# apple/ml-mdm

Hardware: AMD Instinct MI355X
Metric: denoise-steps/sec, whole job = N x optimizer steps/s at per-GPU batch 64 (train fwd+bwd+optimizer, cc12m_64x64 U-Net) (higher is better)
Workload: dtype bf16; 1 GPU; unet64 train step, per-GPU batch 64, global batch 64; global_batch=64, parallelism=dp1, settle_steps=15

## Files before the change

### include/mdm_hip_ext.h

```cpp
#ifndef MDM_HIP_EXT_H_
#define MDM_HIP_EXT_H_
#ifdef __cplusplus
extern "C" {
#endif

int mdm_attn_cross_bias(const void* qkv, const void* kvc, const float* mask, const float* bias, int bias_ld,
                        const void* base, int base_ld, void* out, int B, int L, int S, int H, int d, int dtype,
                        void* stream);

int mdm_attn_cross_maps(const void* qkv, const void* kvc, const float* mask, const float* bias, int bias_ld, float* acc,
                        int acc_ld, float w_host, const float* w_dev, int B, int L, int S, int H, int d, int dtype,
                        void* stream);

int mdm_attn_cross_maps_bwd(const void* qkv, const void* kvc, const float* mask, const float* dacc, int dacc_ld, float w,
                            void* dq, size_t dq_bs, int dq_rs, int B, int L, int S, int H, int d, int dtype, void* stream);

int mdm_freeu_plan(int N, int H, int W, int C1, int C2, int dtype, int structure, size_t* ws_bytes);
int mdm_freeu_stats(const void* h, const void* r, void* ws, size_t ws_bytes, int N, int H, int W, int C1, int C2,
                    int structure, int dtype, void* stream);
int mdm_freeu_apply(const void* h, const void* r, const void* ws, size_t ws_bytes, void* out, int N, int H, int W, int C1,
                    int C2, float b, float s, int structure, int dtype, void* stream);

int mdm_cfg_plan(int B, size_t chw, int rescale_on, size_t* ws_bytes);
int mdm_cfg_stats(const float* x_t, const float* pred, const float* pred_uncond, const float* gamma, const float* run_prev,
// ... 10 lines not shown

int mdm_abs_quantile_plan(int B, size_t n, size_t* ws_bytes);
int mdm_abs_quantile(const float* x, void* ws, size_t ws_bytes, int B, size_t n, float q, float cmin, float cmax, float* thr,
                     float* stats, void* stream);

int mdm_t5_attn_fwd_lse(const void* qkv, const int* seq_start, const int* pos, const float* bias_table, void* out, float* lse,
                        int B, int T, int S, int max_len, int H, int d, int dtype, void* stream);
int mdm_t5_attn_bwd(const void* qkv, const void* out, const float* lse, const void* dout, const int* seq_start, const int* pos,
                    const float* bias_table, void* dqkv, int B, int T, int S, int max_len, int H, int d, int dtype,
                    void* stream);
int mdm_t5_gated_gelu_bwd(const void* u, const void* dy, void* du, int T, int F, int dtype, void* stream);
int mdm_t5_rms_bwd(const float* x, const float* ln_w, const void* dh, float* dx, void* dx_lo, int T, int D, float eps,
                   int dtype, void* stream);
int mdm_t5_final_rms_bwd(const float* x, const void* delta, const float* ln_w, const float* dout, const int* flat, float* dx,
                         void* dx_lo, int T, int D, float eps, int dtype, void* stream);
int mdm_t5_embed_rms_slots(const int* ids, const float* table, const int* slot_of_id, const float* learned, const float* ln_w,
                           float* x, void* h, int T, int D, int vocab, int n_ids, int P, float eps, int dtype, void* stream);
int mdm_t5_embed_bwd(const float* dx0, const int* slot_start, const int* tokens, float* dlearned, int P, int D, int n, int T,
                     void* stream);

int mdm_sampler_step_sa(const float* x_t, const float* pred, const float* pred_uncond, float guidance, const float* gamma,
                        const float* gamma_last, const float* gamma_h0, const float* gamma_h1, const float* gate,
                        const float* thr, const float* noise, const unsigned long long* rng_state, int rng_stream, float* h0,
                        float* h1, float* psum, float* x0_out, float* x_last_out, int B, size_t chw, int pred_type, int clip,
                        float image_scale, int max_predictor, int max_corrector, void* stream);

int mdm_sampler_invert_step(const float* x_s, const float* pred, const float* pred_uncond, float guidance,
                            const float* gamma_s, const float* gamma_t, float* x_t_out, int B, size_t chw, int pred_type,
                            void* stream);
int mdm_sampler_noise_map(const float* x_t, const float* x_s, const float* pred, const float* pred_uncond, float guidance,
                          const float* gamma, const float* gamma_last, const float* thr, float* z_out, int B, size_t chw,
                          int pred_type, int mode, float ddim_eta, int clip, float image_scale, void* stream);

#ifdef __cplusplus
}
#endif
#endif
```

### ml-mdm_amd/csrc/gemm_conv.hip

```cpp
#include <stdio.h>
#include <stdlib.h>

#include <type_traits>
#include <utility>

#include "common.hpp"
#include "conv_args.hpp"

namespace mdm {



__device__ __forceinline__ void load4(const float* p, float (&o)[4]) {
  const f32x4 t = *reinterpret_cast<const f32x4*>(p);
  o[0] = t[0]; o[1] = t[1]; o[2] = t[2]; o[3] = t[3];
}
__device__ __forceinline__ void load4(const bf16* p, float (&o)[4]) {
  const bf16x4 t = *reinterpret_cast<const bf16x4*>(p);
  o[0] = (float)t[0]; o[1] = (float)t[1]; o[2] = (float)t[2]; o[3] = (float)t[3];
}

__device__ __attribute__((aligned(16))) uint4 g_zero_page[4] = {};


// ... 1096 lines not shown
}

template <int MODE, int BIG>
__global__ __launch_bounds__(BIG ? 512 : 256, 2) void conv_wgrad_bl_kernel(WgradArgs p, WgradGroup gr) {
#if defined(__HIP_DEVICE_COMPILE__)
  typedef bf16 T;
  constexpr int EPV = 8, BKM = 64;
  constexpr int NTHR = BIG ? 512 : 256;
  constexpr int BM = BIG ? 256 : 128, BN = BM;
  constexpr int TM = BIG ? 128 : 64, TN = 64, MT = TM / 16, NT = 4;
  constexpr int ROWB = BM * 2;
  constexpr int CPRW = ROWB / 16;
  constexpr int RPP = NTHR / CPRW;
  constexpr int A_BYTES = BKM * ROWB, STAGE = 2 * A_BYTES;
  constexpr int NWN = BIG ? 4 : 2;
  constexpr int KS1 = 32 * ROWB;
  constexpr unsigned INVALID = 0x7F000000u;
  constexpr int WAITN = 2 * (MT + NT - 1) > 15 ? 15 : 2 * (MT + NT - 1);
  extern __shared__ __attribute__((aligned(16))) char smem[];

  const int tid = threadIdx.x, lane = tid & 63, wave = tid >> 6;
  const int wm = wave / NWN, wn = wave % NWN;
  const int quad = lane >> 4, l16 = lane & 15;

  const int tiles_k = (p.K + BN - 1) / BN;
  const int tiles_n = (p.Cout + BM - 1) / BM;
  const int tiles = tiles_k * tiles_n;
  int lid = xcd_remap(blockIdx.x, gridDim.x);
  int grp = 0;
  if (p.groups > 0) { grp = lid / (tiles * p.splits); lid -= grp * tiles * p.splits; }
  const int split = lid / tiles;
  const int t = lid - split * tiles;
  const int n0 = (t / tiles_k) * BM, k0 = (t % tiles_k) * BN;
  if (MODE == MODE_3x3 && p.skip_cout > 0) {
    const int ph = n0 / p.skip_cout, tp = k0 / p.Cin;
    const int dj = tp / 3 - (ph >> 1), dk = tp % 3 - (ph & 1);
    if ((unsigned)dj > 1u || (unsigned)dk > 1u) return;
  }
  const void* const x_ptr = p.groups > 0 ? gr.x[grp] : p.x;
  const void* const dy_ptr = p.groups > 0 ? gr.dy[grp] : p.dy;

  const int ps = tid % CPRW;
  const int srow = tid / CPRW;
  const int lc = ((((ps >> 1) ^ tr_swz(srow)) << 1) | (ps & 1));
  const int a_col = n0 + lc * EPV;
  const int kk = k0 + lc * EPV;
  int tap = 0, cin = kk;
  if (MODE != MODE_1x1) { tap = kk / p.Cin; cin = kk - tap * p.Cin; }
  const int kh = (tap * 11) >> 5, kw = tap - 3 * kh;
  const unsigned bias = MODE == MODE_3x3 ? (unsigned)(p.W + 1) * p.Cin * 2u : 0u;
  unsigned a_vo[4], b_vo[4];
#pragma unroll
  for (int j = 0; j < 4; ++j) {
    const unsigned r = j * RPP + srow;
    a_vo[j] = a_col < p.Cout ? (r * p.Cout + a_col) * 2u : INVALID;
    b_vo[j] = kk < p.K ? (r * p.Cin + cin) * 2u + (MODE == MODE_3x3 ? (unsigned)(kh * p.W + kw) * p.Cin * 2u : 0u) : INVALID;
  }
  const unsigned a_bytes = (unsigned)p.M * p.Cout * 2u;
  const unsigned b_bytes = (unsigned)p.N * p.H * p.W * p.Cin * 2u + bias;
  char* const a_base = const_cast<char*>(reinterpret_cast<const char*>(dy_ptr));
  char* const b_base = const_cast<char*>(reinterpret_cast<const char*>(x_ptr)) - bias;
  const int wave_lds = __builtin_amdgcn_readfirstlane(wave * 1024);
  const int logW = 31 - __builtin_clz(p.W);

  const int mt_begin = split * p.mtiles_per_split;
  const int mt_total = (p.M + BKM - 1) / BKM;
// ... 2 lines not shown

#define MDM_BLDS(rs, lds_off, voff, soff)                                                                   \
  __builtin_amdgcn_raw_ptr_buffer_load_lds(rs, (__attribute__((address_space(3))) void*)(lds_off), 16, voff, soff, 0, 0)
#define MDM_WG_TILE_STATE(it_)                                                                              \
  const bool more_ = (it_) < nt;                                                                            \
  const auto rsA = __builtin_amdgcn_make_buffer_rsrc(a_base, 0, more_ ? a_bytes : 0u, 0x00020000);         \
  const auto rsB = __builtin_amdgcn_make_buffer_rsrc(b_base, 0, more_ ? b_bytes : 0u, 0x00020000);         \
  const int mb_ = (mt_begin + (it_)) * BKM;                                                                 \
  const int a_soff = mb_ * p.Cout * 2, b_soff = mb_ * p.Cin * 2;
#define MDM_WG_PIECE(stage, q)                                                                              \
  {                                                                                                         \
    constexpr int j_ = (q) >> 1;                                                                            \
    const int m_ = mb_ + j_ * RPP + srow;                                                                   \
    bool v_ = m_ < p.M;                                                                                     \
    if (((q) & 1) == 0) {                                                                                   \
      MDM_BLDS(rsA, (stage) + j_ * (RPP * ROWB) + wave_lds, v_ ? a_vo[j_] : INVALID, a_soff);               \
    } else {                                                                                                \
      if (MODE == MODE_3x3) {                                                                               \
        const int ow_ = m_ & (p.W - 1), oh_ = (m_ >> logW) & (p.H - 1);                                     \
        v_ = v_ && (unsigned)(oh_ + kh - 1) < (unsigned)p.H && (unsigned)(ow_ + kw - 1) < (unsigned)p.W;    \
      }                                                                                                     \
      MDM_BLDS(rsB, (stage) + A_BYTES + j_ * (RPP * ROWB) + wave_lds, v_ ? b_vo[j_] : INVALID, b_soff);     \
    }                                                                                                       \
  }

  f32x4 acc[MT][NT];
#pragma unroll
  for (int i = 0; i < MT; ++i)
#pragma unroll
    for (int j = 0; j < NT; ++j) acc[i][j] = f32x4{0.f, 0.f, 0.f, 0.f};
  const int bias_k0 = (MODE == MODE_3x3 && p.skip_cout > 0) ? (((n0 / p.skip_cout) >> 1) * 3 + ((n0 / p.skip_cout) & 1)) * p.Cin : 0;
  constexpr int BR = MT / NWN;
  const int wn_s = __builtin_amdgcn_readfirstlane(wn);
  const int bias_share = p.groups > 0 ? 1 : p.bias_share;
  const int kt_rel = k0 >= bias_k0 ? (k0 - bias_k0) / BN : bias_share;
  const bool bias_blk = (p.groups > 0 ? gr.bout[grp] != nullptr : p.bslab != nullptr) && kt_rel < bias_share;
  const int bias_chunk = (nt + bias_share - 1) / bias_share;
  const int bias_b0 = bias_blk ? min(kt_rel * bias_chunk, nt) : nt;
  const int bias_b1 = bias_blk ? min(bias_b0 + bias_chunk, nt) : nt;

  unsigned fa[MT], fb[NT];
  {
    const unsigned smem_base = (unsigned)(size_t)(__attribute__((address_space(3))) char*)smem;
    const int r0 = quad * 8 + (l16 >> 2);
    const int fsw = (l16 >> 2) | ((quad & 1) << 2);
#pragma unroll
    for (int c = 0; c < MT; ++c) fa[c] = smem_base + r0 * ROWB + (((wm * MT + c) ^ fsw) << 5) + ((l16 & 3) << 3);
#pragma unroll
    for (int c = 0; c < NT; ++c) fb[c] = smem_base + A_BYTES + r0 * ROWB + (((wn * NT + c) ^ fsw) << 5) + ((l16 & 3) << 3);
  }

  if (nt > 0) {
    {
      MDM_WG_TILE_STATE(0);
      MDM_WG_PIECE(smem, 0); MDM_WG_PIECE(smem, 1); MDM_WG_PIECE(smem, 2); MDM_WG_PIECE(smem, 3);
      MDM_WG_PIECE(smem, 4); MDM_WG_PIECE(smem, 5); MDM_WG_PIECE(smem, 6); MDM_WG_PIECE(smem, 7);
    }
    {
      MDM_WG_TILE_STATE(1);
      MDM_WG_PIECE(smem + STAGE, 0); MDM_WG_PIECE(smem + STAGE, 1); MDM_WG_PIECE(smem + STAGE, 2); MDM_WG_PIECE(smem + STAGE, 3);
      MDM_WG_PIECE(smem + STAGE, 4); MDM_WG_PIECE(smem + STAGE, 5); MDM_WG_PIECE(smem + STAGE, 6); MDM_WG_PIECE(smem + STAGE, 7);
    }
    asm volatile("s_waitcnt vmcnt(0)" ::: "memory");
    __syncthreads();
    u32x2 ra[MT][2], rb0[NT][2], rb1[NT][2];
#pragma unroll
    for (int c = 0; c < NT; ++c) MDM_TR2(rb0[c][0], rb0[c][1], fb[c], 0);
#pragma unroll
    for (int c = 0; c < MT; ++c) MDM_TR2(ra[c][0], ra[c][1], fa[c], 0);
// ... 29 lines not shown
      char* const dst = smem + so;                                                                          \
      _Pragma("unroll") for (int c = 0; c < NT; ++c) { const unsigned ad = fb[c] + sn; MDM_TR2(rb0[c][0], rb0[c][1], ad, 0); } \
      _Pragma("unroll") for (int j = 0; j < NT; ++j) bq[j] = frag_of(rb1[j][0], rb1[j][1]);                 \
      _Pragma("unroll") for (int i = 0; i < MT; ++i) {                                                      \
        const Frag<T> aq = frag_of(ra[i][0], ra[i][1]);                                                     \
        _Pragma("unroll") for (int j = 0; j < NT; ++j) mma16(acc[i][j], bq[j], aq);                         \
        if (BIAS && i / BR == wn_s) bsum[i % BR] = frag_sum_guarded(aq, bsum[i % BR]);                      \
        if (MT == 8) { MDM_WG_PIECE_RT(dst, i) } else { MDM_WG_PIECE_RT(dst, 2 * i) MDM_WG_PIECE_RT(dst, 2 * i + 1) } \
        { const unsigned ad = fa[i] + sn; MDM_TR2(ra[i][0], ra[i][1], ad, 0); }                             \
        __builtin_amdgcn_sched_barrier(0);                                                                  \
      }                                                                                                     \
    }
#define MDM_WG_PIECE_RT(stage, q)                                                                           \
    switch (q) {                                                                                            \
      case 0: MDM_WG_PIECE(stage, 0) break; case 1: MDM_WG_PIECE(stage, 1) break;                           \
      case 2: MDM_WG_PIECE(stage, 2) break; case 3: MDM_WG_PIECE(stage, 3) break;                           \
      case 4: MDM_WG_PIECE(stage, 4) break; case 5: MDM_WG_PIECE(stage, 5) break;                           \
      case 6: MDM_WG_PIECE(stage, 6) break; default: MDM_WG_PIECE(stage, 7) break;                          \
    }
    int it = 0;
    float bsum[BR];
    for (; it < bias_b0; ++it) MDM_WG_ITER(false)
#pragma unroll
    for (int i = 0; i < BR; ++i) bsum[i] = 0.f;
    for (; it < bias_b1; ++it) MDM_WG_ITER(true)
    if (bias_blk) {
#pragma unroll
      for (int r = 0; r < BR; ++r) {
        float v = bsum[r];
        v += __shfl_xor(v, 16, 64);
        v += __shfl_xor(v, 32, 64);
        const int n = n0 + wm * TM + (wn * BR + r) * 16 + l16;
        if (quad == 0 && n < p.Cout) {
          if (p.groups > 0) gr.bout[grp][n] += v;
          else p.bslab[((size_t)split * bias_share + kt_rel) * p.Cout + n] = v;
        }
      }
    }
    for (; it < nt; ++it) MDM_WG_ITER(false)
    asm volatile("s_waitcnt vmcnt(0) lgkmcnt(0)" ::: "memory");
#undef MDM_WG_PIECE_RT
#undef MDM_WG_ITER
  } else if (bias_blk && p.groups == 0 && quad == 0) {
#pragma unroll
    for (int r = 0; r < BR; ++r) {
      const int n = n0 + wm * TM + (wn * BR + r) * 16 + l16;
      if (n < p.Cout) p.bslab[((size_t)split * bias_share + kt_rel) * p.Cout + n] = 0.f;
    }
  }
#undef MDM_WG_PIECE
#undef MDM_WG_TILE_STATE
#undef MDM_BLDS

  if (bias_blk && p.groups == 0 && split == 0 && kt_rel == 0 && n0 == 0 && tid == 0)
    reinterpret_cast<int*>(p.bslab - WG_BHDR)[0] = bias_share;
  const bool direct = p.groups > 0;
  float* __restrict__ S = direct ? gr.out[grp] : p.slab + (size_t)split * p.Cout * p.K;
  const bool vec_ok = (p.K & 3) == 0;
  if (!direct) {
#pragma unroll
    for (int i = 0; i < MT; ++i) {
      const int n = n0 + wm * TM + i * 16 + l16;
      if (n >= p.Cout) continue;
#pragma unroll
      for (int j = 0; j < NT; ++j) {
        const int k = k0 + wn * TN + j * 16 + quad * 4;
        if (k >= p.K) continue;
        float* o = S + (size_t)n * p.K + k;
        if (vec_ok) {
          *reinterpret_cast<f32x4*>(o) = acc[i][j];
        } else {
#pragma unroll
          for (int e = 0; e < 4; ++e) if (k + e < p.K) o[e] = acc[i][j][e];
        }
      }
    }
  } else if (vec_ok && n0 + BM <= p.Cout && k0 + BN <= p.K) {
    float* const o0 = S + (size_t)(n0 + wm * TM + l16) * p.K + k0 + wn * TN + quad * 4;
    f32x4 old[2][NT];
#pragma unroll
    for (int j = 0; j < NT; ++j) old[0][j] = *reinterpret_cast<const f32x4*>(o0 + j * 16);
#pragma unroll
    for (int i = 0; i < MT; ++i) {
      if (i + 1 < MT) {
#pragma unroll
        for (int j = 0; j < NT; ++j) old[(i + 1) & 1][j] = *reinterpret_cast<const f32x4*>(o0 + (size_t)(i + 1) * 16 * p.K + j * 16);
      }
#pragma unroll
      for (int j = 0; j < NT; ++j) *reinterpret_cast<f32x4*>(o0 + (size_t)i * 16 * p.K + j * 16) = old[i & 1][j] + acc[i][j];
    }
  } else {
#pragma unroll
    for (int i = 0; i < MT; ++i) {
      const int n = n0 + wm * TM + i * 16 + l16;
      if (n >= p.Cout) continue;
#pragma unroll
      for (int j = 0; j < NT; ++j) {
        const int k = k0 + wn * TN + j * 16 + quad * 4;
        if (k >= p.K) continue;
        float* o = S + (size_t)n * p.K + k;
#pragma unroll
        for (int e = 0; e < 4; ++e) if (k + e < p.K) o[e] += acc[i][j][e];
      }
    }
  }
#endif
}
#undef MDM_TR2

template <int NT>
__device__ __forceinline__ void wgrad_bias_reduce(const float* __restrict__ bslab, float* __restrict__ dbias, int splits,
                                                  int Cout, int accumulate, int blk, float* lds) {
  constexpr int G = NT / 32;
  const int tid = threadIdx.x, c = tid & 31, g = tid >> 5;
  const int rows = splits * reinterpret_cast<const int*>(bslab - WG_BHDR)[0];
  const int o = blk * 32 + c;
  float s0 = 0.f, s1 = 0.f, s2 = 0.f, s3 = 0.f;
  if (o < Cout) {
    const float* src = bslab + o;
    int r = g;
    for (; r + 3 * G < rows; r += 4 * G) {
      s0 += src[(size_t)r * Cout];
      s1 += src[(size_t)(r + G) * Cout];
      s2 += src[(size_t)(r + 2 * G) * Cout];
      s3 += src[(size_t)(r + 3 * G) * Cout];
    }
    for (; r < rows; r += G) s0 += src[(size_t)r * Cout];
  }
  lds[tid] = (s0 + s1) + (s2 + s3);
  __syncthreads();
  if (g == 0 && o < Cout) {
    float s = lds[c];
#pragma unroll
    for (int q = 1; q < G; ++q) s += lds[q * 32 + c];
    dbias[o] = accumulate ? dbias[o] + s : s;
  }
}

__global__ __launch_bounds__(192) void wgrad_reduce_kernel(const float* __restrict__ slab, float* __restrict__ dw,
                                                           const float* __restrict__ bslab, float* __restrict__ dbias,
                                                           int splits, int Cout, int Cin, int taps, int accumulate,
                                                           int bblocks) {
  __shared__ float tile[64 * 9 + 4];
  const int tid = threadIdx.x;
  if ((int)blockIdx.x < bblocks) {
    wgrad_bias_reduce<192>(bslab, dbias, splits, Cout, accumulate, (int)blockIdx.x, tile);
    return;
  }
  const int wb = (int)blockIdx.x - bblocks;
  const int iblocks = (Cin + 63) / 64;
  const int o = wb / iblocks, i0 = (wb - o * iblocks) * 64;
  const int ni = min(64, Cin - i0);
  const size_t total = (size_t)Cout * Cin * taps;
  const int K = Cin * taps;
  const int per_o = taps * 16;
  if (tid < per_o) {
    const int tp = tid >> 4, i4 = (tid & 15) * 4;
    f32x4 acc[8];
#pragma unroll
    for (int u = 0; u < 8; ++u) acc[u] = f32x4{0.f, 0.f, 0.f, 0.f};
    if (i4 < ni) {
      const float* src = slab + (size_t)o * K + (size_t)tp * Cin + i0 + i4;
      int sp = 0;
      for (; sp + 8 <= splits; sp += 8) {
#pragma unroll
        for (int u = 0; u < 8; ++u) acc[u] += *reinterpret_cast<const f32x4*>(src + (size_t)(sp + u) * total);
      }
      for (; sp < splits; ++sp) acc[0] += *reinterpret_cast<const f32x4*>(src + (size_t)sp * total);
    }
    const f32x4 s4 = ((acc[0] + acc[1]) + (acc[2] + acc[3])) + ((acc[4] + acc[5]) + (acc[6] + acc[7]));
#pragma unroll
    for (int q = 0; q < 4; ++q) tile[(i4 + q) * taps + tp] = s4[q];
  }
  __syncthreads();
  const int run = ni * taps;
  float* const dst = dw + ((size_t)o * Cin + i0) * taps;
  for (int r = tid; r < run; r += 192) dst[r] = accumulate ? dst[r] + tile[r] : tile[r];
}

__global__ __launch_bounds__(256) void wgrad_reduce_flat_kernel(const float* __restrict__ slab, float* __restrict__ dw,
                                                                const float* __restrict__ bslab,
                                                                float* __restrict__ dbias, int splits, int Cout,
                                                                size_t total, int accumulate, int wblocks, int bblocks) {
  if ((int)blockIdx.x < bblocks) {
    __shared__ float part[256];
    wgrad_bias_reduce<256>(bslab, dbias, splits, Cout, accumulate, (int)blockIdx.x, part);
    return;
  }
  const size_t n4 = total / 4;
  const f32x4* s4 = reinterpret_cast<const f32x4*>(slab);
  f32x4* d4 = reinterpret_cast<f32x4*>(dw);
  for (size_t i = (size_t)(blockIdx.x - bblocks) * 256 + threadIdx.x; i < n4; i += (size_t)wblocks * 256) {
    f32x4 a0 = s4[i], a1 = {0.f, 0.f, 0.f, 0.f}, a2 = a1, a3 = a1;
    int sp = 1;
    for (; sp + 4 <= splits; sp += 4) {
      a0 += s4[(size_t)sp * n4 + i];
      a1 += s4[(size_t)(sp + 1) * n4 + i];
      a2 += s4[(size_t)(sp + 2) * n4 + i];
      a3 += s4[(size_t)(sp + 3) * n4 + i];
    }
    for (; sp < splits; ++sp) a0 += s4[(size_t)sp * n4 + i];
    const f32x4 a = (a0 + a1) + (a2 + a3);
    d4[i] = accumulate ? d4[i] + a : a;
  }
}

template <typename T>
__global__ void pack_weight_kernel(const float* __restrict__ w, T* __restrict__ wf, T* __restrict__ wd,
                                   int Cout, int Cin, int taps, int Cin_pad, int Cout_pad, int kbf, int kbd) {
  const size_t Kf = (size_t)taps * Cin_pad, Kd = (size_t)taps * Cout_pad;
  const size_t total_f = (size_t)Cout * Kf;
  const size_t total_d = wd ? (size_t)Cin * Kd : 0;
  for (size_t idx = (size_t)blockIdx.x * blockDim.x + threadIdx.x; idx < total_f + total_d;
       idx += (size_t)gridDim.x * blockDim.x) {
    if (idx < total_f) {
      const int o = (int)(idx / Kf);
      const int kpos = (int)(idx - (size_t)o * Kf);
      int tp, i;
      if (kbf) { const int cb = kpos / (taps * kbf), r = kpos - cb * taps * kbf; tp = r / kbf; i = cb * kbf + (r - tp * kbf); }
      else { tp = kpos / Cin_pad; i = kpos - tp * Cin_pad; }
      wf[idx] = from_f32<T>(i < Cin ? w[((size_t)o * Cin + i) * taps + tp] : 0.f);
    } else {
      const size_t d = idx - total_f;
      const int i = (int)(d / Kd);
      const int kpos = (int)(d - (size_t)i * Kd);
      int tp, o;
      if (kbd) { const int ob = kpos / (taps * kbd), r = kpos - ob * taps * kbd; tp = r / kbd; o = ob * kbd + (r - tp * kbd); }
      else { tp = kpos / Cout_pad; o = kpos - tp * Cout_pad; }
      wd[d] = from_f32<T>(o < Cout ? w[((size_t)o * Cin + i) * taps + (taps - 1 - tp)] : 0.f);
    }
  }
}

template <typename T, int TAPS>
__global__ __launch_bounds__(256) void pack_weight_tiled_kernel(const float* __restrict__ w, T* __restrict__ wf,
                                                                T* __restrict__ wd, int Cout, int Cin, int kbf,
                                                                int kbd) {
// ... 1109 lines not shown

extern "C" int mdm_conv_wgrad_grouped(const void* const* x, const void* const* dy, float* const* dw,
                                      float* const* dbias, int groups, int M, int Cin, int Cout, int dtype,
                                      void* stream) {
  MDM_CHECK_ARG(x && dy && dw && groups >= 1 && groups <= WG_MAXG);
  MDM_CHECK_ARG(dtype == DT_BF16 && Cin % 8 == 0 && Cout % 8 == 0 && M > 0);
  WgradArgs a = {};
  a.N = M; a.H = 1; a.W = 1; a.Cin = Cin; a.Ho = 1; a.Wo = 1; a.Cout = Cout; a.stride = 1;
  a.M = M; a.K = Cin; a.splits = 1; a.groups = groups;
  a.mtiles_per_split = (M + 63) / 64;
  MDM_CHECK_ARG(wgrad_bl_ok(a, 1));
  WgradGroup gr = {};
  for (int g = 0; g < groups; ++g) {
    MDM_CHECK_ARG(x[g] && dy[g] && dw[g]);
    gr.x[g] = x[g]; gr.dy[g] = dy[g]; gr.out[g] = dw[g]; gr.bout[g] = dbias ? dbias[g] : nullptr;
  }
  int te = wgrad_group_tile(M, Cout, Cin, groups);
  if (!te) te = wgrad_forced_tile(Cout, Cin, DT_BF16);
  if (!te) te = (Cout >= 192 && Cin >= 192) ? 256 : 128;
  const int tiles = ((Cout + te - 1) / te) * ((Cin + te - 1) / te);
  hipStream_t st = reinterpret_cast<hipStream_t>(stream);
  constexpr int smem = 4 * 128 * 128, smem_big = 4 * 64 * 512;
  if (te == 256) {
    ensure_dynamic_lds(conv_wgrad_bl_kernel<MODE_1x1, 1>, smem_big);
    hipLaunchKernelGGL((conv_wgrad_bl_kernel<MODE_1x1, 1>), dim3(tiles * groups), dim3(512), smem_big, st, a, gr);
  } else {
    ensure_dynamic_lds(conv_wgrad_bl_kernel<MODE_1x1, 0>, smem);
    hipLaunchKernelGGL((conv_wgrad_bl_kernel<MODE_1x1, 0>), dim3(tiles * groups), dim3(256), smem, st, a, gr);
  }
  MDM_NOTE_KERNEL("conv_wgrad_bl_kernel<%d, %d>", MODE_1x1, te == 256 ? 1 : 0);
  MDM_LAUNCH_STATUS();
}

extern "C" int mdm_conv_wgrad_reduce(const float* ws, float* dw_oihw, float* dbias, const void* dy, int M, int Cin,
                                     int Cout, int ksize, int accumulate, int dtype, void* stream) {
  MDM_CHECK_ARG(ws && dw_oihw && (ksize == 1 || ksize == 3));
  const int K = ksize * ksize * Cin;
  int splits; size_t wsb;
  int rc = mdm_conv_wgrad_plan(M, Cout, K, dtype, &splits, &wsb);
  if (rc) return rc;
  hipStream_t st = reinterpret_cast<hipStream_t>(stream);
  float* const bias_ws = const_cast<float*>(ws) + (size_t)splits * Cout * K;
  const float* bslab = (dbias && dtype == DT_BF16) ? bias_ws + WG_BHDR : nullptr;
  const int bblocks = bslab ? (Cout + 31) / 32 : 0;
  if (ksize == 1) {
    const size_t total = (size_t)Cout * Cin;
    const int wblocks = (int)((total / 4 + 255) / 256 > 2048 ? 2048 : (total / 4 + 255) / 256);
    hipLaunchKernelGGL(wgrad_reduce_flat_kernel, dim3(wblocks + bblocks), dim3(256), 0, st, ws, dw_oihw, bslab, dbias,
                       splits, Cout, total, accumulate, wblocks, bblocks);
  } else {
    const int wblocks = Cout * ((Cin + 63) / 64);
    hipLaunchKernelGGL(wgrad_reduce_kernel, dim3(wblocks + bblocks), dim3(192), 0, st, ws, dw_oihw, bslab, dbias,
                       splits, Cout, Cin, ksize * ksize, accumulate, bblocks);
  }
  if (dbias && !bslab) {
    MDM_CHECK_ARG(dy);
    return mdm_colsum(dy, dbias, bias_ws, M, Cout, accumulate, dtype, stream);
  }
  MDM_LAUNCH_STATUS();
}

extern "C" int mdm_pack_weight(const float* w_oihw, void* w_fwd, void* w_dgrad, int Cout, int Cin, int ksize,
                               int Cin_pad, int Cout_pad, int kblock_fwd, int kblock_dgrad, int dtype,
                               void* stream) {
  MDM_CHECK_ARG(w_oihw && w_fwd);
  MDM_CHECK_ARG(ksize == 1 || ksize == 3);
// ... 72 lines not shown
```

### ml-mdm_amd/mdm_hip/ops.py

```python
import ctypes
import weakref

import torch

from . import _lib
from . import tiling as _tiling

F32, BF16, F32_SPLIT, F32_SPLIT_W = 0, 1, 2, 3

_fp32_split = False
_weight_planes_on = True


class fp32_split:

    def __init__(self, enabled: bool = True):
        global _fp32_split
        self._prev = _fp32_split
        _fp32_split = bool(enabled)

    def __enter__(self):
        return self

    def __exit__(self, *a):
# ... 119 lines not shown
        torch.cuda.current_stream().wait_stream(_side_stream)
    _side_keep.clear()


def _off_critical_path(tensors, fn):
    if not (_async_wgrad and _grad_sink is not None):
        return fn()
    side = side_stream()
    if _raw_stream is None:
        side.wait_stream(torch.cuda.current_stream())
        with torch.cuda.stream(side):
            fn()
            done = torch.cuda.Event()
            done.record(side)
    else:
        cur = _current_stream_obj()
        side.wait_stream(cur)
        torch.cuda.set_stream(side)
        try:
            fn()
            done = torch.cuda.Event()
            done.record(side)
        finally:
            torch.cuda.set_stream(cur)
    live = [t for t in tensors if t is not None]
    _side_keep.append((done, live))
    if len(_side_keep) >= 64:
        _side_keep[:] = [e for e in _side_keep if not e[0].query()]


_defer_wgrad = False
_wgrad_queue = {}
_WG_MAX = 32


def enable_deferred_wgrad(flag: bool, max_group: int = 32):
    global _defer_wgrad, _WG_MAX
    flush_wgrad_queue()
    _defer_wgrad = bool(flag)
    _WG_MAX = max(1, min(32, int(max_group)))


def wgrad_grouped(xs, dys, dws, dbs=None):
    G = len(xs)
    M, cin = xs[0].shape
    cout = dys[0].shape[1]
    for t in list(xs) + list(dys):
        _require_gpu(t)
    xs, dys = [_c(t) for t in xs], [_c(t) for t in dys]
    arr = lambda vals: (ctypes.c_void_p * G)(*vals)
    _lib.check(_lib.lib().mdm_conv_wgrad_grouped(arr([_p(t) for t in xs]), arr([_p(t) for t in dys]), arr([_p(t) for t in dws]),
                                                 arr([_p(t) for t in dbs]) if dbs is not None else None, G, M, cin, cout,
                                                 _dt(xs[0]), _stream()), "mdm_conv_wgrad_grouped")


def _queue_wgrad(x, dy, weight, bias, slot, bslot, M, cin, cout):
    key = (M, cin, cout, x.device.index)
    q = _wgrad_queue.setdefault(key, [])
    q.append((x, dy, weight, bias, slot, bslot))
    _sink_defer(weight)
    if bslot is not None:
        _sink_defer(bias)
    if len(q) == _WG_MAX:
        _flush_key(key)


def _flush_key(key):
    q = _wgrad_queue.pop(key, None)
    if not q:
        return
    M, cin, cout, _ = key
    L = _lib.lib()
    tile = ctypes.c_int(0)
    _lib.check(L.mdm_conv_wgrad_group_plan(M, cout, cin, BF16, len(q), ctypes.byref(tile)), "mdm_conv_wgrad_group_plan")
    tensors = [t for e in q for t in (e[0], e[1])]
    if tile.value and all((e[5] is not None) == (q[0][5] is not None) for e in q):
        G = len(q)
        arr = lambda vals: (ctypes.c_void_p * G)(*vals)
        xs, dys, dws = arr([_p(e[0]) for e in q]), arr([_p(e[1]) for e in q]), arr([_p(e[4]) for e in q])
        dbs = arr([_p(e[5]) for e in q]) if q[0][5] is not None else None

        def go():
            _prof_wrap("conv_wgrad grouped x%d M=%d N=%d K=%d" % (G, M, cout, cin), 2.0 * G * M * cout * cin, lambda: _lib.check(
                L.mdm_conv_wgrad_grouped(xs, dys, dws, dbs, G, M, cin, cout, BF16, _stream()), "mdm_conv_wgrad_grouped"))
            for e in q:
                _grad_sink.ready(e[2])
                if e[5] is not None:
                    _grad_sink.ready(e[3])
    else:
        def go():
            for x, dy, w, b, slot, bslot in q:
                _wgrad_launch(x, dy, M, 1, 1, cin, 1, 1, cout, 1, 1, out=slot, dbias=bslot)
                _grad_sink.ready(w)
                if bslot is not None:
                    _grad_sink.ready(b)

    _off_critical_path(tensors, go)


def flush_wgrad_queue():
    for key in list(_wgrad_queue):
        _flush_key(key)
    flush_gn_params()


_gn_pending = []
_gn_pool = {}
_gn_tables = {}


def _gn_rows(N, C, device):
    ent = _gn_pool.get(device.index)
    need = 2 * N * C
    if ent is None or ent[1] + need > ent[0].numel():
        size = max(need, 0 if ent is None else 2 * ent[0].numel(), 16 << 20)
        ent = _gn_pool[device.index] = [torch.empty(size, dtype=torch.float32, device=device), 0]
    off = ent[1]
    ent[1] = off + need
    return ent[0][off:off + N * C], ent[0][off + N * C:off + need]


def flush_gn_params():
    if not _gn_pending:
        return
    dev = _gn_pending[0][0].device
# ... 9 lines not shown
            blocks += (C + 255) // 256
        table = torch.from_numpy(rec.view(np.uint8).copy()).to(dev)
        if len(_gn_tables) > 64:
            _gn_tables.clear()
        ent = _gn_tables[key] = (table, blocks)
    table, blocks = ent
    _lib.check(_lib.lib().mdm_gn_param_reduce_multi(_p(table), len(key), blocks, _stream()), "mdm_gn_param_reduce_multi")
    for e in _gn_pending:
        _grad_sink.ready(e[6])
        _grad_sink.ready(e[7])
    _gn_pending.clear()
    for ent in _gn_pool.values():
        ent[1] = 0


class _FlushPointFn(torch.autograd.Function):

    @staticmethod
    def forward(ctx, x):
        return x.view_as(x)

    @staticmethod
    def backward(ctx, dy):
        flush_wgrad_queue()
        return dy


def wgrad_flush_point(x):
    return _FlushPointFn.apply(x) if (_defer_wgrad and x.requires_grad) else x


def _wgrad_into_sink(x, dy, weight, bias, slot, bslot, N, H, W, cin, Ho, Wo, cout, ks, stride):
    M = N * Ho * Wo
    if _defer_wgrad and _async_wgrad and ks == 1 and x.dtype == torch.bfloat16 and M >= 4096:
        _queue_wgrad(x.reshape(M, cin), dy.reshape(M, cout), weight, bias, slot, bslot, M, cin, cout)
        return

    def go():
        _wgrad_launch(x, dy, N, H, W, cin, Ho, Wo, cout, ks, stride, out=slot, dbias=bslot)
        _grad_sink.ready(weight)
        if bslot is not None:
            _grad_sink.ready(bias)

    _off_critical_path((x, dy), go)


def _cache_slot(weight):
    k = id(weight)
    ent = _wcache.get(k)
    if ent is None or ent[0]() is not weight:
        ent = (weakref.ref(weight, lambda _r, k=k: _wcache.pop(k, None)), {})
        _wcache[k] = ent
    return ent[1]


def _round_up(v, m):
    return (v + m - 1) // m * m


def packed_weight(weight: torch.Tensor, bias, dtype: torch.dtype, forward_only: bool = False):
    key = (dtype, "fwd") if forward_only else dtype
    ent = _cache_slot(weight)
    ver = (weight._version, None if bias is None else bias._version, weight.data_ptr(), _pack_epoch)
    if key in ent and ent[key][0] == ver:
        return ent[key][1]
    _require_gpu(weight)
    L = _lib.lib()
    cout, cin = weight.shape[0], weight.shape[1]
    ks = weight.shape[2] if weight.dim() == 4 else 1
# ... 2593 lines not shown
```

Baseline: 11.66 steps/s.

## Group deferred 3x3 and split-K 1x1 weight-gradient GEMMs into batched launches

Extends deferred weight-gradient grouping to handle 3x3 stride-1 convolutions and 1x1 convs the old plan rejected, using a new grouped split-M kernel path with per-group slabs and a multi-group reduce kernel. A cost model picks the tile and split count, and decides whether grouping beats issuing separate launches. The aim is to cut launch count and fill the CUs better for small wgrad GEMMs. It adds workspace slab traffic and a reduce pass, and the 3x3 path is gated so high-resolution layers get a group cap of 0 by default.

```diff
diff --git a/include/mdm_hip_ext.h b/include/mdm_hip_ext.h
--- a/include/mdm_hip_ext.h
+++ b/include/mdm_hip_ext.h
@@ -66,6 +66,12 @@
                           const float* gamma, const float* gamma_last, const float* thr, float* z_out, int B, size_t chw,
                           int pred_type, int mode, float ddim_eta, int clip, float image_scale, void* stream);
 
+int mdm_conv_wgrad_group_plan2(int M, int Cout, int K, int ksize, int groups, int* tile_out, int* splits_out,
+                               size_t* ws_bytes, int* pays_out);
+int mdm_conv_wgrad_grouped_split(const void* const* x, const void* const* dy, float* const* dw, float* const* dbias,
+                                 int groups, int N, int H, int W, int Cin, int Cout, int ksize, int splits, float* ws,
+                                 int accumulate, int dtype, void* stream);
+
 #ifdef __cplusplus
 }
 #endif
diff --git a/ml-mdm_amd/csrc/gemm_conv.hip b/ml-mdm_amd/csrc/gemm_conv.hip
--- a/ml-mdm_amd/csrc/gemm_conv.hip
+++ b/ml-mdm_amd/csrc/gemm_conv.hip
@@ -1152,6 +1152,8 @@
   const int split = lid / tiles;
   const int t = lid - split * tiles;
   const int n0 = (t / tiles_k) * BM, k0 = (t % tiles_k) * BN;
+  const bool direct = p.groups > 0 && p.slab == nullptr;
+  const int sidx = grp * p.splits + split;
   if (MODE == MODE_3x3 && p.skip_cout > 0) {
     const int ph = n0 / p.skip_cout, tp = k0 / p.Cin;
     const int dj = tp / 3 - (ph >> 1), dk = tp % 3 - (ph & 1);
@@ -1220,9 +1222,9 @@
   const int bias_k0 = (MODE == MODE_3x3 && p.skip_cout > 0) ? (((n0 / p.skip_cout) >> 1) * 3 + ((n0 / p.skip_cout) & 1)) * p.Cin : 0;
   constexpr int BR = MT / NWN;
   const int wn_s = __builtin_amdgcn_readfirstlane(wn);
-  const int bias_share = p.groups > 0 ? 1 : p.bias_share;
+  const int bias_share = direct ? 1 : p.bias_share;
   const int kt_rel = k0 >= bias_k0 ? (k0 - bias_k0) / BN : bias_share;
-  const bool bias_blk = (p.groups > 0 ? gr.bout[grp] != nullptr : p.bslab != nullptr) && kt_rel < bias_share;
+  const bool bias_blk = (direct ? gr.bout[grp] != nullptr : p.bslab != nullptr) && kt_rel < bias_share;
   const int bias_chunk = (nt + bias_share - 1) / bias_share;
   const int bias_b0 = bias_blk ? min(kt_rel * bias_chunk, nt) : nt;
   const int bias_b1 = bias_blk ? min(bias_b0 + bias_chunk, nt) : nt;
@@ -1318,8 +1320,8 @@
         v += __shfl_xor(v, 32, 64);
         const int n = n0 + wm * TM + (wn * BR + r) * 16 + l16;
         if (quad == 0 && n < p.Cout) {
-          if (p.groups > 0) gr.bout[grp][n] += v;
-          else p.bslab[((size_t)split * bias_share + kt_rel) * p.Cout + n] = v;
+          if (direct) gr.bout[grp][n] += v;
+          else p.bslab[((size_t)sidx * bias_share + kt_rel) * p.Cout + n] = v;
         }
       }
     }
@@ -1327,21 +1329,20 @@
     asm volatile("s_waitcnt vmcnt(0) lgkmcnt(0)" ::: "memory");
 #undef MDM_WG_PIECE_RT
 #undef MDM_WG_ITER
-  } else if (bias_blk && p.groups == 0 && quad == 0) {
+  } else if (bias_blk && !direct && quad == 0) {
 #pragma unroll
     for (int r = 0; r < BR; ++r) {
       const int n = n0 + wm * TM + (wn * BR + r) * 16 + l16;
-      if (n < p.Cout) p.bslab[((size_t)split * bias_share + kt_rel) * p.Cout + n] = 0.f;
+      if (n < p.Cout) p.bslab[((size_t)sidx * bias_share + kt_rel) * p.Cout + n] = 0.f;
     }
   }
 #undef MDM_WG_PIECE
 #undef MDM_WG_TILE_STATE
 #undef MDM_BLDS
 
-  if (bias_blk && p.groups == 0 && split == 0 && kt_rel == 0 && n0 == 0 && tid == 0)
+  if (bias_blk && !direct && sidx == 0 && kt_rel == 0 && n0 == 0 && tid == 0)
     reinterpret_cast<int*>(p.bslab - WG_BHDR)[0] = bias_share;
-  const bool direct = p.groups > 0;
-  float* __restrict__ S = direct ? gr.out[grp] : p.slab + (size_t)split * p.Cout * p.K;
+  float* __restrict__ S = direct ? gr.out[grp] : p.slab + (size_t)sidx * p.Cout * p.K;
   const bool vec_ok = (p.K & 3) == 0;
   if (!direct) {
 #pragma unroll
@@ -1395,11 +1396,10 @@
 #undef MDM_TR2
 
 template <int NT>
-__device__ __forceinline__ void wgrad_bias_reduce(const float* __restrict__ bslab, float* __restrict__ dbias, int splits,
+__device__ __forceinline__ void wgrad_bias_reduce(const float* __restrict__ bslab, float* __restrict__ dbias, int rows,
                                                   int Cout, int accumulate, int blk, float* lds) {
   constexpr int G = NT / 32;
   const int tid = threadIdx.x, c = tid & 31, g = tid >> 5;
-  const int rows = splits * reinterpret_cast<const int*>(bslab - WG_BHDR)[0];
   const int o = blk * 32 + c;
   float s0 = 0.f, s1 = 0.f, s2 = 0.f, s3 = 0.f;
   if (o < Cout) {
@@ -1423,17 +1423,9 @@
   }
 }
 
-__global__ __launch_bounds__(192) void wgrad_reduce_kernel(const float* __restrict__ slab, float* __restrict__ dw,
-                                                           const float* __restrict__ bslab, float* __restrict__ dbias,
-                                                           int splits, int Cout, int Cin, int taps, int accumulate,
-                                                           int bblocks) {
-  __shared__ float tile[64 * 9 + 4];
+__device__ __forceinline__ void wgrad_reduce_tr_block(const float* __restrict__ slab, float* __restrict__ dw, int splits,
+                                                      int Cout, int Cin, int taps, int accumulate, int wb, float* tile) {
   const int tid = threadIdx.x;
-  if ((int)blockIdx.x < bblocks) {
-    wgrad_bias_reduce<192>(bslab, dbias, splits, Cout, accumulate, (int)blockIdx.x, tile);
-    return;
-  }
-  const int wb = (int)blockIdx.x - bblocks;
   const int iblocks = (Cin + 63) / 64;
   const int o = wb / iblocks, i0 = (wb - o * iblocks) * 64;
   const int ni = min(64, Cin - i0);
@@ -1464,19 +1456,25 @@
   for (int r = tid; r < run; r += 192) dst[r] = accumulate ? dst[r] + tile[r] : tile[r];
 }
 
-__global__ __launch_bounds__(256) void wgrad_reduce_flat_kernel(const float* __restrict__ slab, float* __restrict__ dw,
-                                                                const float* __restrict__ bslab,
-                                                                float* __restrict__ dbias, int splits, int Cout,
-                                                                size_t total, int accumulate, int wblocks, int bblocks) {
+__global__ __launch_bounds__(192) void wgrad_reduce_kernel(const float* __restrict__ slab, float* __restrict__ dw,
+                                                           const float* __restrict__ bslab, float* __restrict__ dbias,
+                                                           int splits, int Cout, int Cin, int taps, int accumulate,
+                                                           int bblocks) {
+  __shared__ float tile[64 * 9 + 4];
   if ((int)blockIdx.x < bblocks) {
-    __shared__ float part[256];
-    wgrad_bias_reduce<256>(bslab, dbias, splits, Cout, accumulate, (int)blockIdx.x, part);
+    const int rows = splits * reinterpret_cast<const int*>(bslab - WG_BHDR)[0];
+    wgrad_bias_reduce<192>(bslab, dbias, rows, Cout, accumulate, (int)blockIdx.x, tile);
     return;
   }
+  wgrad_reduce_tr_block(slab, dw, splits, Cout, Cin, taps, accumulate, (int)blockIdx.x - bblocks, tile);
+}
+
+__device__ __forceinline__ void wgrad_reduce_flat_block(const float* __restrict__ slab, float* __restrict__ dw, int splits,
+                                                        size_t total, int accumulate, int wb, int wblocks) {
   const size_t n4 = total / 4;
   const f32x4* s4 = reinterpret_cast<const f32x4*>(slab);
   f32x4* d4 = reinterpret_cast<f32x4*>(dw);
-  for (size_t i = (size_t)(blockIdx.x - bblocks) * 256 + threadIdx.x; i < n4; i += (size_t)wblocks * 256) {
+  for (size_t i = (size_t)wb * 256 + threadIdx.x; i < n4; i += (size_t)wblocks * 256) {
     f32x4 a0 = s4[i], a1 = {0.f, 0.f, 0.f, 0.f}, a2 = a1, a3 = a1;
     int sp = 1;
     for (; sp + 4 <= splits; sp += 4) {
@@ -1489,6 +1487,46 @@
     const f32x4 a = (a0 + a1) + (a2 + a3);
     d4[i] = accumulate ? d4[i] + a : a;
   }
+}
+
+__global__ __launch_bounds__(256) void wgrad_reduce_flat_kernel(const float* __restrict__ slab, float* __restrict__ dw,
+                                                                const float* __restrict__ bslab,
+                                                                float* __restrict__ dbias, int splits, int Cout,
+                                                                size_t total, int accumulate, int wblocks, int bblocks) {
+  if ((int)blockIdx.x < bblocks) {
+    __shared__ float part[256];
+    const int rows = splits * reinterpret_cast<const int*>(bslab - WG_BHDR)[0];
+    wgrad_bias_reduce<256>(bslab, dbias, rows, Cout, accumulate, (int)blockIdx.x, part);
+    return;
+  }
+  wgrad_reduce_flat_block(slab, dw, splits, total, accumulate, (int)blockIdx.x - bblocks, wblocks);
+}
+
+struct WgradReduceTable {
+  float* dw[WG_MAXG];
+  float* dbias[WG_MAXG];
+};
+
+template <int TAPS>
+__global__ __launch_bounds__(TAPS == 1 ? 256 : 192) void wgrad_reduce_multi_kernel(const float* __restrict__ slab,
+                                                                                   const float* __restrict__ bslab,
+                                                                                   WgradReduceTable tb, int splits,
+                                                                                   int Cout, int Cin, int accumulate,
+                                                                                   int wblocks, int bblocks) {
+  constexpr int NT = TAPS == 1 ? 256 : 192;
+  __shared__ float lds[TAPS == 1 ? 256 : 64 * 9 + 4];
+  const int per = wblocks + bblocks;
+  const int g = (int)blockIdx.x / per, b = (int)blockIdx.x - g * per;
+  const size_t total = (size_t)Cout * Cin * TAPS;
+  if (b < bblocks) {
+    if (tb.dbias[g] == nullptr) return;
+    const int rows = splits * reinterpret_cast<const int*>(bslab - WG_BHDR)[0];
+    wgrad_bias_reduce<NT>(bslab + (size_t)g * rows * Cout, tb.dbias[g], rows, Cout, accumulate, b, lds);
+    return;
+  }
+  const float* const src = slab + (size_t)g * splits * total;
+  if (TAPS == 1) wgrad_reduce_flat_block(src, tb.dw[g], splits, total, accumulate, b - bblocks, wblocks);
+  else wgrad_reduce_tr_block(src, tb.dw[g], splits, Cout, Cin, TAPS, accumulate, b - bblocks, lds);
 }
 
 template <typename T>
@@ -2664,6 +2702,132 @@
   MDM_LAUNCH_STATUS();
 }
 
+
+static int wgrad_group2_tile(int Cout, int K) {
+  if (const int forced = wgrad_forced_tile(Cout, K, DT_BF16)) return forced;
+  return (Cout >= 192 && K >= 192) ? 256 : 128;
+}
+
+static int wgrad_bias_share(int K, int te) {
+  const int kt = (K + te - 1) / te;
+  return kt < WG_BSHARE ? (kt < 1 ? 1 : kt) : WG_BSHARE;
+}
+
+static double wgrad_group2_choose(int M, int Cout, int K, int ksize, int groups, int te, int* splits_out) {
+  const int mt_total = (M + 63) / 64;
+  const long tiles = (long)((Cout + te - 1) / te) * ((K + te - 1) / te) * groups;
+  const int slots = te == 256 ? device_cus() : 2 * device_cus();
+  const double t_tile = te == 256 ? 1.7 : 1.06, t_fix = te == 256 ? 12.0 : 5.0;
+  const double slab_us = (double)groups * Cout * K * 4.0 / 5.0e6;
+  const double eff = (double)tiles / (double)(((tiles + slots - 1) / slots) * slots);
+  const bool fills = tiles >= (long)(0.7 * slots) && eff >= 0.7;
+  double best = 1e30;
+  int best_s = 1;
+  const int smax = fills ? 1 : (mt_total < 64 ? mt_total : 64);
+  for (int sp = 1; sp <= smax; ++sp) {
+    const int per = (mt_total + sp - 1) / sp;
+    if ((mt_total + per - 1) / per != sp) continue;
+    const double rounds = fills ? (double)tiles / slots > 1.0 ? (double)tiles / slots : 1.0 : (double)((tiles * sp + slots - 1) / slots);
+    const double cost = rounds * (per * t_tile + t_fix) + sp * slab_us + ((sp > 1 || ksize == 3) ? 4.0 : 0.0);
+    if (cost < best) { best = cost; best_s = sp; }
+  }
+  *splits_out = best_s;
+  return best;
+}
+
+static double wgrad_single_cost(int M, int Cout, int K) {
+  int te, sp;
+  wgrad_choose(M, Cout, K, DT_BF16, &te, &sp);
+  const int mt_total = (M + 63) / 64, per = (mt_total + sp - 1) / sp;
+  const long blocks = (long)((Cout + te - 1) / te) * ((K + te - 1) / te) * sp;
+  const int slots = te == 256 ? 256 : 512;
+  return (double)((blocks + slots - 1) / slots) * (per * (te == 256 ? 1.7 : 1.06) + (te == 256 ? 12.0 : 5.0)) +
+         sp * (double)Cout * K * 4.0 / 5.0e6 + (sp > 1 ? 4.0 : 0.0);
+}
+
+extern "C" int mdm_conv_wgrad_group_plan2(int M, int Cout, int K, int ksize, int groups, int* tile_out, int* splits_out,
+                                          size_t* ws_bytes, int* pays_out) {
+  MDM_CHECK_ARG(tile_out && splits_out && ws_bytes && pays_out);
+  MDM_CHECK_ARG(M > 0 && Cout > 0 && K > 0 && (ksize == 1 || ksize == 3) && groups >= 1 && groups <= WG_MAXG);
+  const int te = wgrad_group2_tile(Cout, K);
+  int splits = 1;
+  const double cost = wgrad_group2_choose(M, Cout, K, ksize, groups, te, &splits);
+  *tile_out = te;
+  *splits_out = splits;
+  const size_t brows = (size_t)groups * (splits * WG_BSHARE > 64 ? splits * WG_BSHARE : 64);
+  *ws_bytes = ((size_t)groups * splits * Cout * K + WG_BHDR + brows * Cout) * sizeof(float);
+  *pays_out = groups >= 2 && !wgrad_direct_slabs(M, Cout, K, DT_BF16) && cost < groups * wgrad_single_cost(M, Cout, K);
+  return 0;
+}
+
+extern "C" int mdm_conv_wgrad_grouped_split(const void* const* x, const void* const* dy, float* const* dw,
+                                            float* const* dbias, int groups, int N, int H, int W, int Cin, int Cout,
+                                            int ksize, int splits, float* ws, int accumulate, int dtype, void* stream) {
+  MDM_CHECK_ARG(x && dy && dw && groups >= 1 && groups <= WG_MAXG);
+  MDM_CHECK_ARG(dtype == DT_BF16 && (ksize == 1 || ksize == 3) && Cin % 8 == 0 && Cout % 8 == 0);
+  MDM_CHECK_ARG(N > 0 && H > 0 && W > 0 && (size_t)N * H * W < 0x7FFFFFFFu);
+  WgradArgs a = {};
+  a.N = N; a.H = H; a.W = W; a.Cin = Cin; a.Ho = H; a.Wo = W; a.Cout = Cout; a.stride = 1;
+  a.M = N * H * W; a.K = ksize * ksize * Cin; a.groups = groups;
+  if (ksize == 1) { a.N = a.M; a.H = a.W = a.Ho = a.Wo = 1; }
+  const int mt_total = (a.M + 63) / 64;
+  MDM_CHECK_ARG(splits >= 1 && splits <= mt_total);
+  a.splits = splits;
+  a.mtiles_per_split = (mt_total + splits - 1) / splits;
+  MDM_CHECK_ARG(wgrad_bl_ok(a, ksize));
+  const bool slabs = splits > 1 || ksize == 3 || !accumulate;
+  MDM_CHECK_ARG(!slabs || ws);
+  const int te = wgrad_group2_tile(Cout, a.K);
+  const int tiles = ((Cout + te - 1) / te) * ((a.K + te - 1) / te);
+  WgradGroup gr = {};
+  WgradReduceTable tb = {};
+  for (int g = 0; g < groups; ++g) {
+    MDM_CHECK_ARG(x[g] && dy[g] && dw[g]);
+    gr.x[g] = x[g]; gr.dy[g] = dy[g]; gr.out[g] = dw[g]; gr.bout[g] = dbias ? dbias[g] : nullptr;
+    tb.dw[g] = dw[g]; tb.dbias[g] = gr.bout[g];
+  }
+  if (slabs) {
+    a.slab = ws;
+    a.bias_share = wgrad_bias_share(a.K, te);
+    if (dbias) a.bslab = ws + (size_t)groups * splits * Cout * a.K + WG_BHDR;
+  }
+  hipStream_t st = reinterpret_cast<hipStream_t>(stream);
+  constexpr int smem = 4 * 128 * 128, smem_big = 4 * 64 * 512;
+  const dim3 grid(tiles * splits * groups);
+  if (te == 256) {
+    if (ksize == 1) {
+      ensure_dynamic_lds(conv_wgrad_bl_kernel<MODE_1x1, 1>, smem_big);
+      hipLaunchKernelGGL((conv_wgrad_bl_kernel<MODE_1x1, 1>), grid, dim3(512), smem_big, st, a, gr);
+    } else {
+      ensure_dynamic_lds(conv_wgrad_bl_kernel<MODE_3x3, 1>, smem_big);
+      hipLaunchKernelGGL((conv_wgrad_bl_kernel<MODE_3x3, 1>), grid, dim3(512), smem_big, st, a, gr);
+    }
+  } else {
+    if (ksize == 1) {
+      ensure_dynamic_lds(conv_wgrad_bl_kernel<MODE_1x1, 0>, smem);
+      hipLaunchKernelGGL((conv_wgrad_bl_kernel<MODE_1x1, 0>), grid, dim3(256), smem, st, a, gr);
+    } else {
+      ensure_dynamic_lds(conv_wgrad_bl_kernel<MODE_3x3, 0>, smem);
+      hipLaunchKernelGGL((conv_wgrad_bl_kernel<MODE_3x3, 0>), grid, dim3(256), smem, st, a, gr);
+    }
+  }
+  MDM_NOTE_KERNEL("conv_wgrad_bl_kernel<%d, %d>", ksize == 1 ? MODE_1x1 : MODE_3x3, te == 256 ? 1 : 0);
+  if (slabs) {
+    const int bblocks = a.bslab ? (Cout + 31) / 32 : 0;
+    if (ksize == 1) {
+      const size_t total = (size_t)Cout * Cin;
+      const int wblocks = (int)((total / 4 + 255) / 256 > 2048 ? 2048 : (total / 4 + 255) / 256);
+      hipLaunchKernelGGL(wgrad_reduce_multi_kernel<1>, dim3((wblocks + bblocks) * groups), dim3(256), 0, st, ws, a.bslab, tb,
+                         splits, Cout, Cin, accumulate, wblocks, bblocks);
+    } else {
+      const int wblocks = Cout * ((Cin + 63) / 64);
+      hipLaunchKernelGGL(wgrad_reduce_multi_kernel<9>, dim3((wblocks + bblocks) * groups), dim3(192), 0, st, ws, a.bslab, tb,
+                         splits, Cout, Cin, accumulate, wblocks, bblocks);
+    }
+  }
+  MDM_LAUNCH_STATUS();
+}
+
 extern "C" int mdm_conv_wgrad_reduce(const float* ws, float* dw_oihw, float* dbias, const void* dy, int M, int Cin,
                                      int Cout, int ksize, int accumulate, int dtype, void* stream) {
   MDM_CHECK_ARG(ws && dw_oihw && (ksize == 1 || ksize == 3));
diff --git a/ml-mdm_amd/mdm_hip/ops.py b/ml-mdm_amd/mdm_hip/ops.py
--- a/ml-mdm_amd/mdm_hip/ops.py
+++ b/ml-mdm_amd/mdm_hip/ops.py
@@ -175,6 +175,7 @@
 _defer_wgrad = False
 _wgrad_queue = {}
 _WG_MAX = 32
+_WG_HIRES = 0
 
 
 def enable_deferred_wgrad(flag: bool, max_group: int = 32):
@@ -197,14 +198,18 @@
                                                  _dt(xs[0]), _stream()), "mdm_conv_wgrad_grouped")
 
 
-def _queue_wgrad(x, dy, weight, bias, slot, bslot, M, cin, cout):
-    key = (M, cin, cout, x.device.index)
+def _wgrad_group_cap(ks, H, W):
+    return min(_WG_MAX, _WG_HIRES) if (ks == 3 and H * W >= 4096) else _WG_MAX
+
+
+def _queue_wgrad(x, dy, weight, bias, slot, bslot, ks, N, H, W, cin, cout):
+    key = (ks, N, H, W, cin, cout, x.device.index)
     q = _wgrad_queue.setdefault(key, [])
-    q.append((x, dy, weight, bias, slot, bslot))
+    q.append((_c(x), _c(dy), weight, bias, slot, bslot))
     _sink_defer(weight)
     if bslot is not None:
         _sink_defer(bias)
-    if len(q) == _WG_MAX:
+    if len(q) >= _wgrad_group_cap(ks, H, W):
         _flush_key(key)
 
 
@@ -212,20 +217,33 @@
     q = _wgrad_queue.pop(key, None)
     if not q:
         return
-    M, cin, cout, _ = key
+    ks, N, H, W, cin, cout, _ = key
+    M, G = N * H * W, len(q)
     L = _lib.lib()
-    tile = ctypes.c_int(0)
-    _lib.check(L.mdm_conv_wgrad_group_plan(M, cout, cin, BF16, len(q), ctypes.byref(tile)), "mdm_conv_wgrad_group_plan")
+    tile, splits, wsb, pays = ctypes.c_int(0), ctypes.c_int(1), ctypes.c_size_t(0), ctypes.c_int(0)
+    if ks == 1:
+        _lib.check(L.mdm_conv_wgrad_group_plan(M, cout, cin, BF16, G, ctypes.byref(tile)), "mdm_conv_wgrad_group_plan")
+    nosplit = bool(tile.value)
+    if not nosplit:
+        _lib.check(L.mdm_conv_wgrad_group_plan2(M, cout, ks * ks * cin, ks, G, ctypes.byref(tile), ctypes.byref(splits),
+                                                ctypes.byref(wsb), ctypes.byref(pays)), "mdm_conv_wgrad_group_plan2")
     tensors = [t for e in q for t in (e[0], e[1])]
-    if tile.value and all((e[5] is not None) == (q[0][5] is not None) for e in q):
-        G = len(q)
+    if (nosplit or pays.value) and all((e[5] is not None) == (q[0][5] is not None) for e in q):
         arr = lambda vals: (ctypes.c_void_p * G)(*vals)
         xs, dys, dws = arr([_p(e[0]) for e in q]), arr([_p(e[1]) for e in q]), arr([_p(e[4]) for e in q])
         dbs = arr([_p(e[5]) for e in q]) if q[0][5] is not None else None
+        dev = q[0][0].device
 
         def go():
-            _prof_wrap("conv_wgrad grouped x%d M=%d N=%d K=%d" % (G, M, cout, cin), 2.0 * G * M * cout * cin, lambda: _lib.check(
-                L.mdm_conv_wgrad_grouped(xs, dys, dws, dbs, G, M, cin, cout, BF16, _stream()), "mdm_conv_wgrad_grouped"))
+            if not nosplit:
+                ws = _f32_ws(wsb.value, dev) if (splits.value > 1 or ks == 3) else None
+                _prof_wrap("conv_wgrad grouped x%d /%d %dx%d M=%d N=%d K=%d" % (G, splits.value, ks, ks, M, cout, ks * ks * cin),
+                           2.0 * G * M * cout * ks * ks * cin, lambda: _lib.check(
+                    L.mdm_conv_wgrad_grouped_split(xs, dys, dws, dbs, G, N, H, W, cin, cout, ks, splits.value, _p(ws), 1, BF16,
+                                                   _stream()), "mdm_conv_wgrad_grouped_split"))
+            else:
+                _prof_wrap("conv_wgrad grouped x%d M=%d N=%d K=%d" % (G, M, cout, cin), 2.0 * G * M * cout * cin, lambda: _lib.check(
+                    L.mdm_conv_wgrad_grouped(xs, dys, dws, dbs, G, M, cin, cout, BF16, _stream()), "mdm_conv_wgrad_grouped"))
             for e in q:
                 _grad_sink.ready(e[2])
                 if e[5] is not None:
@@ -233,7 +251,7 @@
     else:
         def go():
             for x, dy, w, b, slot, bslot in q:
-                _wgrad_launch(x, dy, M, 1, 1, cin, 1, 1, cout, 1, 1, out=slot, dbias=bslot)
+                _wgrad_launch(x, dy, N, H, W, cin, H, W, cout, ks, 1, out=slot, dbias=bslot)
                 _grad_sink.ready(w)
                 if bslot is not None:
                     _grad_sink.ready(b)
@@ -309,9 +327,14 @@
 
 def _wgrad_into_sink(x, dy, weight, bias, slot, bslot, N, H, W, cin, Ho, Wo, cout, ks, stride):
     M = N * Ho * Wo
-    if _defer_wgrad and _async_wgrad and ks == 1 and x.dtype == torch.bfloat16 and M >= 4096:
-        _queue_wgrad(x.reshape(M, cin), dy.reshape(M, cout), weight, bias, slot, bslot, M, cin, cout)
-        return
+    if _defer_wgrad and _async_wgrad and x.dtype == torch.bfloat16 and M >= 4096:
+        if ks == 1:
+            _queue_wgrad(x, dy, weight, bias, slot, bslot, 1, M, 1, 1, cin, cout)
+            return
+        if ks == 3 and stride == 1 and not (H & (H - 1)) and not (W & (W - 1)) and min(cin, cout) >= 128 \
+                and _wgrad_group_cap(3, H, W) >= 2:
+            _queue_wgrad(x, dy, weight, bias, slot, bslot, 3, N, H, W, cin, cout)
+            return
 
     def go():
         _wgrad_launch(x, dy, N, H, W, cin, Ho, Wo, cout, ks, stride, out=slot, dbias=bslot)
```

Result: no change. 11.73 steps/s, median of 6 (+0.5%).
